# zqqqqz2000/MixGRPO

Measured on AMD Instinct MI355X. Metric: GRPO train-step images/sec, FLUX.1-dev 1024^2, higher is better.
Workload: dtype bf16

## Files before the change

mixgrpo_amd/csrc/attention_bwd.hip:

```cpp
#include "../../include/mixgrpo_hip.h"
#include "attn_fp8_quant.h"
#include "attn_operands.h"
#include "common.h"

#include <cstdlib>
#include <type_traits>

namespace {

constexpr int HD = 128;

__device__ __forceinline__ int rm_off(int row, int chunk) { return row * 256 + ((chunk ^ (row & 15)) << 4); }
__device__ __forceinline__ int t64_off(int d, int slot) { return d * 128 + ((slot ^ ((d >> 1) & 7)) << 4); }
__device__ __forceinline__ int t32_off(int d, int slot) { return d * 64 + ((slot ^ (((d >> 2) ^ (d >> 1)) & 3)) << 4); }

typedef __attribute__((ext_vector_type(4))) unsigned int u32x4;
__device__ __forceinline__ auto buf_rsrc(const void* p, long bytes) {
  const unsigned n = bytes > 0xfffffff0L ? 0xfffffff0u : (unsigned)bytes;
  return __builtin_amdgcn_make_buffer_rsrc(const_cast<void*>(p), 0, (int)n, 0x00020000);
}
template <typename R>
__device__ __forceinline__ uint4 buf_ld16(R rs, unsigned voff, unsigned soff) {
  const u32x4 v = __builtin_amdgcn_raw_buffer_load_b128(rs, (int)voff, (int)soff, 0);
  return make_uint4(v.x, v.y, v.z, v.w);
}
template <typename R>
__device__ __forceinline__ float buf_ld_f32(R rs, unsigned voff, unsigned soff) {
  return __builtin_bit_cast(float, __builtin_amdgcn_raw_buffer_load_b32(rs, (int)voff, (int)soff, 0));
}

__global__ void __launch_bounds__(256) attn_bwd_prep_kernel(const bf16_raw* __restrict__ O, const bf16_raw* __restrict__ dO,
                                                            long ldo, long o_bstride, float* __restrict__ delta,
                                                            bf16_raw* __restrict__ dOt, int H, int S, int Sp, int valid) {
  __shared__ bf16_raw tile[64][130];
  const int lane = threadIdx.x & 63, w = threadIdx.x >> 6;
  const int hh = blockIdx.y, b = blockIdx.z, t0 = blockIdx.x * 64;
  for (int i = 0; i < 16; ++i) {
    const int tl = w * 16 + i, s = t0 + tl;
    uint32_t ud = 0;
    float acc = 0.f;
    if (s < valid) {
      const long off = (long)b * o_bstride + (long)s * ldo + hh * HD + 2 * lane;
      ud = *reinterpret_cast<const uint32_t*>(dO + off);
      const uint32_t uo = *reinterpret_cast<const uint32_t*>(O + off);
      acc = bf2f(ud & 0xffff) * bf2f(uo & 0xffff) + bf2f(ud >> 16) * bf2f(uo >> 16);
    }
    *reinterpret_cast<uint32_t*>(&tile[tl][2 * lane]) = ud;
    acc = wave_sum(acc);
    if (lane == 0 && s < S) delta[((long)b * H + hh) * S + s] = acc;
  }
  __syncthreads();
  for (int id = threadIdx.x; id < 128 * 8; id += 256) {
    const int d = id >> 3, c = id & 7;
    bf16_raw* dst = dOt + (((long)b * H + hh) * HD + d) * Sp + t0 + c * 8;
    if (t0 + c * 8 < Sp) {
      uint4 u;
      u.x = (uint32_t)tile[c * 8 + 0][d] | ((uint32_t)tile[c * 8 + 1][d] << 16);
      u.y = (uint32_t)tile[c * 8 + 2][d] | ((uint32_t)tile[c * 8 + 3][d] << 16);
      u.z = (uint32_t)tile[c * 8 + 4][d] | ((uint32_t)tile[c * 8 + 5][d] << 16);
      u.w = (uint32_t)tile[c * 8 + 6][d] | ((uint32_t)tile[c * 8 + 7][d] << 16);
      *reinterpret_cast<uint4*>(dst) = u;
    }
  }
}

struct BwdArgs {
  const bf16_raw* Q;
  const bf16_raw* K;
  const bf16_raw* V;
  const bf16_raw* Qt;
  const bf16_raw* Kt;
  const bf16_raw* dO;
  const bf16_raw* dOt;
  const float* lse;
  const float* delta;
  bf16_raw* dQ;
  bf16_raw* dK;
  bf16_raw* dV;
  int B, H, S, Sp;
  long ldo, o_bstride;
  float scale, scale_log2e, neg_inv_scale;
  int kv_len;
};

constexpr int DKV_STAGE = 4 * 8192 + 256;
__global__ void __launch_bounds__(512, 2) attn_bwd_dkv_kernel(BwdArgs g) {
  extern __shared__ __attribute__((aligned(16))) char smem[];
  const int tid = threadIdx.x, lane = tid & 63, wid = tid >> 6;
  const int r = lane & 31, h = lane >> 5;
  const int nkb = (g.S + 255) / 256;
  int bid = blockIdx.x;
  xcd_remap(bid, nkb * g.H * g.B);
  const int kt = bid % nkb, bh = bid / nkb;
  const int b = bh / g.H, hh = bh - b * g.H;
  const long bhS = (long)bh * g.S;
  const bf16_raw* Qp = g.Q + bhS * HD;
  const bf16_raw* Qtp = g.Qt + (long)bh * HD * g.Sp;
  const bf16_raw* dOtp = g.dOt + (long)bh * HD * g.Sp;
  const bf16_raw* dOp = g.dO + (long)b * g.o_bstride + hh * HD;

  const int key0 = kt * 256 + wid * 32;
  int krow = key0 + r;
  const bool key_valid = krow < g.S;
  if (krow >= g.S) krow = g.S - 1;
  s16x8 kf[8];
  char* vfrag = smem + 2 * DKV_STAGE + wid * 8192 + lane * 16;
#pragma unroll
  for (int ks = 0; ks < 8; ++ks) {
    kf[ks] = *reinterpret_cast<const s16x8*>(g.K + (bhS + krow) * HD + ks * 16 + h * 8);
    *reinterpret_cast<s16x8*>(vfrag + ks * 1024) =
        *reinterpret_cast<const s16x8*>(g.V + (bhS + krow) * HD + ks * 16 + h * 8);
  }
  f32x16 dv[4], dk[4];
#pragma unroll
  for (int dt = 0; dt < 4; ++dt)
#pragma unroll
    for (int i = 0; i < 16; ++i) dv[dt][i] = dk[dt][i] = 0.f;

  const int s_row = tid >> 4, s_chunk = tid & 15;
  const int s_d = tid >> 2, s_c16 = tid & 3;
  uint4 rq, rdo, rqt, rdot;
  float rl = 0.f;
  const int nqt = (g.S + 31) / 32;
  const auto rs_q = buf_rsrc(Qp, (long)g.S * HD * 2);
  const auto rs_do = buf_rsrc(dOp, ((long)(g.S - 1) * g.ldo + HD) * 2);
  const auto rs_qt = buf_rsrc(Qtp, (long)HD * g.Sp * 2);
  const auto rs_dot = buf_rsrc(dOtp, (long)HD * g.Sp * 2);
  const auto rs_lse = buf_rsrc(g.lse + bhS, (long)g.S * 4);
  const auto rs_dlt = buf_rsrc(g.delta + bhS, (long)g.S * 4);
  const unsigned vo_q = (unsigned)(s_row * HD + s_chunk * 8) * 2, vo_do = (unsigned)(s_row * g.ldo + s_chunk * 8) * 2;
  const unsigned vo_t = (unsigned)(s_d * g.Sp + s_c16 * 8) * 2, vo_l = (unsigned)(tid & 31) * 4;
  float rl2 = 0.f;
  const bool wave0 = __builtin_amdgcn_readfirstlane(wid) == 0;
  const float inv_scale = 1.0f / g.scale;
#define DKV_LOAD(t)                                                                                   \
  do {                                                                                                \
    const unsigned q_base = (unsigned)(t) * 32;                                                       \
    rq = buf_ld16(rs_q, vo_q, q_base * (HD * 2));                                                     \
    rdo = buf_ld16(rs_do, vo_do, q_base * (unsigned)(g.ldo * 2));                                     \
    rqt = buf_ld16(rs_qt, vo_t, q_base * 2);                                                          \
    rdot = buf_ld16(rs_dot, vo_t, q_base * 2);                                                        \
                                                          \
    if (wave0) {           \
      rl = buf_ld_f32(rs_lse, vo_l, q_base * 4);                                                      \
      rl2 = buf_ld_f32(rs_dlt, vo_l, q_base * 4);                                                     \
    }                                                                                                 \
  } while (0)
#define DKV_STORE(buf)                                                                                \
  do {                                                                                                \
    char* base = smem + (buf) * DKV_STAGE;                                                            \
    *reinterpret_cast<uint4*>(base + rm_off(s_row, s_chunk)) = rq;                                    \
    *reinterpret_cast<uint4*>(base + 8192 + rm_off(s_row, s_chunk)) = rdo;                            \
     \
    *reinterpret_cast<uint2*>(base + 16384 + t32_off(s_d, (s_c16 >> 1) * 2) + (s_c16 & 1) * 8) = make_uint2(rqt.x, rqt.y);     \
    *reinterpret_cast<uint2*>(base + 16384 + t32_off(s_d, (s_c16 >> 1) * 2 + 1) + (s_c16 & 1) * 8) = make_uint2(rqt.z, rqt.w); \
    *reinterpret_cast<uint2*>(base + 24576 + t32_off(s_d, (s_c16 >> 1) * 2) + (s_c16 & 1) * 8) = make_uint2(rdot.x, rdot.y);   \
    *reinterpret_cast<uint2*>(base + 24576 + t32_off(s_d, (s_c16 >> 1) * 2 + 1) + (s_c16 & 1) * 8) = make_uint2(rdot.z, rdot.w); \
      \
    if (wave0)                                                                                        \
      reinterpret_cast<float*>(base + 32768)[tid] =                                                   \
          (tid < 32) ? ((nt_ * 32 + tid < g.S) ? -rl * inv_scale : -INFINITY) : -rl2;                 \
  } while (0)

  DKV_LOAD(0);
  { const int nt_ = 0; DKV_STORE(0); }
  __syncthreads();
#pragma unroll
  for (int ks = 0; ks < 8; ++ks) asm volatile("" :: "v"(kf[ks]));
  int cur = 0;
  auto tile = [&](int t, auto mask_tag) __attribute__((always_inline)) {
    constexpr bool MASK = decltype(mask_tag)::value;
    const char* base = smem + cur * DKV_STAGE;
    const float* nls = reinterpret_cast<const float*>(base + 32768);
    const float* ndl = nls + 32;
    f32x16 s, dp;
#pragma unroll
    for (int j = 0; j < 4; ++j) {
      const float4 a = *reinterpret_cast<const float4*>(nls + 8 * j + 4 * h);
      const float4 b2 = *reinterpret_cast<const float4*>(ndl + 8 * j + 4 * h);
      s[4 * j] = a.x; s[4 * j + 1] = a.y; s[4 * j + 2] = a.z; s[4 * j + 3] = a.w;
      dp[4 * j] = b2.x; dp[4 * j + 1] = b2.y; dp[4 * j + 2] = b2.z; dp[4 * j + 3] = b2.w;
    }
    {
      s16x8 qa[2], da[2], vk;
      qa[0] = *reinterpret_cast<const s16x8*>(base + rm_off(r, h));
      da[0] = *reinterpret_cast<const s16x8*>(base + 8192 + rm_off(r, h));
#pragma unroll
      for (int ks = 0; ks < 8; ++ks) {
        vk = *reinterpret_cast<const s16x8*>(vfrag + ks * 1024);
        if (ks + 1 < 8) {
          qa[(ks + 1) & 1] = *reinterpret_cast<const s16x8*>(base + rm_off(r, (ks + 1) * 2 + h));
          da[(ks + 1) & 1] = *reinterpret_cast<const s16x8*>(base + 8192 + rm_off(r, (ks + 1) * 2 + h));
        }
        __builtin_amdgcn_sched_barrier(0);
        s = __builtin_amdgcn_mfma_f32_32x32x16_bf16(qa[ks & 1], kf[ks], s, 0, 0, 0);
        dp = __builtin_amdgcn_mfma_f32_32x32x16_bf16(da[ks & 1], vk, dp, 0, 0, 0);
        __builtin_amdgcn_sched_barrier(0);
      }
    }
    if (t + 1 < nqt) DKV_LOAD(t + 1);
    uint32_t pb[8], dsb[8];
#pragma unroll
    for (int i = 0; i < 16; i += 2) {
      float p0 = __builtin_amdgcn_exp2f(s[i] * g.scale_log2e);
      float p1 = __builtin_amdgcn_exp2f(s[i + 1] * g.scale_log2e);
      if (MASK && !key_valid) p0 = p1 = 0.f;
      const float d0 = p0 * dp[i] * g.scale;
      const float d1 = p1 * dp[i + 1] * g.scale;
      pb[i >> 1] = pack_bf16(p0, p1);
      dsb[i >> 1] = pack_bf16(d0, d1);
    }
    {
      s16x8 pf[2], df[2];
#pragma unroll
      for (int s2 = 0; s2 < 2; ++s2) {
        pf[s2] = __builtin_bit_cast(s16x8, make_uint4(pb[4 * s2], pb[4 * s2 + 1], pb[4 * s2 + 2], pb[4 * s2 + 3]));
        df[s2] = __builtin_bit_cast(s16x8, make_uint4(dsb[4 * s2], dsb[4 * s2 + 1], dsb[4 * s2 + 2], dsb[4 * s2 + 3]));
      }
      auto frag = [&](int i) __attribute__((always_inline)) {
        const int s2 = i >> 3, dt = (i >> 1) & 3, which = i & 1;
        return *reinterpret_cast<const s16x8*>(base + (which ? 16384 : 24576) + t32_off(dt * 32 + r, s2 * 2 + h));
      };
      s16x8 fr[3];
      fr[0] = frag(0); fr[1] = frag(1);
#pragma unroll
      for (int i = 0; i < 16; ++i) {
        if (i + 2 < 16) fr[(i + 2) % 3] = frag(i + 2);
        __builtin_amdgcn_sched_barrier(0);
        const int s2 = i >> 3, dt = (i >> 1) & 3;
        if (i & 1) dk[dt] = __builtin_amdgcn_mfma_f32_32x32x16_bf16(fr[i % 3], df[s2], dk[dt], 0, 0, 0);
        else dv[dt] = __builtin_amdgcn_mfma_f32_32x32x16_bf16(fr[i % 3], pf[s2], dv[dt], 0, 0, 0);
        __builtin_amdgcn_sched_barrier(0);
      }
    }
    if (t + 1 < nqt) { const int nt_ = t + 1; DKV_STORE(cur ^ 1); }
    __syncthreads();
    cur ^= 1;
  };
  if (key0 + 32 > g.S) {
    for (int t = 0; t < nqt; ++t) tile(t, std::true_type{});
  } else {
    for (int t = 0; t < nqt; ++t) tile(t, std::false_type{});
  }
  const int key = key0 + r;
  if (key < g.S) {
    bf16_raw* dkp = g.dK + (bhS + key) * HD;
    bf16_raw* dvp = g.dV + (bhS + key) * HD;
#pragma unroll
    for (int dt = 0; dt < 4; ++dt)
#pragma unroll
      for (int i4 = 0; i4 < 4; ++i4) {
        const int d = dt * 32 + 8 * i4 + 4 * h;
        *reinterpret_cast<uint2*>(dkp + d) = make_uint2(pack_bf16(dk[dt][4 * i4], dk[dt][4 * i4 + 1]),
                                                        pack_bf16(dk[dt][4 * i4 + 2], dk[dt][4 * i4 + 3]));
        *reinterpret_cast<uint2*>(dvp + d) = make_uint2(pack_bf16(dv[dt][4 * i4], dv[dt][4 * i4 + 1]),
                                                        pack_bf16(dv[dt][4 * i4 + 2], dv[dt][4 * i4 + 3]));
      }
  }
}

constexpr int DQ_STAGE = 3 * 16384;
__global__ void __launch_bounds__(512, 2) attn_bwd_dq_kernel(BwdArgs g) {
  extern __shared__ __attribute__((aligned(16))) char smem[];
  const int tid = threadIdx.x, lane = tid & 63, wid = tid >> 6;
  const int r = lane & 31, h = lane >> 5;
  const int nq = (g.S + 255) / 256;
  int bid = blockIdx.x;
  xcd_remap(bid, nq * g.H * g.B);
  const int qt = bid % nq, bh = bid / nq;
  const int b = bh / g.H, hh = bh - b * g.H;
  const long bhS = (long)bh * g.S;
  const bf16_raw* Kp = g.K + bhS * HD;
  const bf16_raw* Vp = g.V + bhS * HD;
  const bf16_raw* Ktp = g.Kt + (long)bh * HD * g.Sp;

  const int q0 = qt * 256 + wid * 32;
  int qrow = q0 + r;
  const bool q_valid = qrow < g.S;
  if (qrow >= g.S) qrow = g.S - 1;
  s16x8 qf[8], dof[8];
  const bf16_raw* dOp = g.dO + (long)b * g.o_bstride + (long)qrow * g.ldo + hh * HD;
#pragma unroll
  for (int ks = 0; ks < 8; ++ks) {
    qf[ks] = *reinterpret_cast<const s16x8*>(g.Q + (bhS + qrow) * HD + ks * 16 + h * 8);
    dof[ks] = *reinterpret_cast<const s16x8*>(dOp + ks * 16 + h * 8);
  }
  const float lse2 = g.lse[bhS + qrow] * 1.4426950408889634f;
  const float dlt = g.delta[bhS + qrow];
  f32x16 dq[4];
#pragma unroll
  for (int dt = 0; dt < 4; ++dt)
#pragma unroll
    for (int i = 0; i < 16; ++i) dq[dt][i] = 0.f;

  const int kc_key0 = tid >> 4, kc_chunk = tid & 15;
  const int vc_d0 = tid >> 3, vc_chunk = tid & 7;
  uint4 sk0, sk1, sv0, sv1, st0, st1;
  const int ntiles = (g.S + 63) / 64;
  const auto rs_k = buf_rsrc(Kp, (long)g.S * HD * 2);
  const auto rs_v = buf_rsrc(Vp, (long)g.S * HD * 2);
  const auto rs_kt = buf_rsrc(Ktp, (long)HD * g.Sp * 2);
  const unsigned vo_k = (unsigned)(kc_key0 * HD + kc_chunk * 8) * 2, vo_kt = (unsigned)(vc_d0 * g.Sp + vc_chunk * 8) * 2;
#define DQ_LOAD(t)                                                                                  \
  do {                                                                                              \
    const unsigned key_base = (unsigned)(t) * 64;                                                   \
    sk0 = buf_ld16(rs_k, vo_k, key_base * (HD * 2));                                                \
    sk1 = buf_ld16(rs_k, vo_k, (key_base + 32) * (HD * 2));                                         \
    sv0 = buf_ld16(rs_v, vo_k, key_base * (HD * 2));                                                \
    sv1 = buf_ld16(rs_v, vo_k, (key_base + 32) * (HD * 2));                                         \
    st0 = buf_ld16(rs_kt, vo_kt, key_base * 2);                                                     \
    st1 = buf_ld16(rs_kt, vo_kt + (unsigned)(64 * g.Sp * 2), key_base * 2);                         \
  } while (0)
#define DQ_STORE(buf)                                                                               \
  do {                                                                                              \
    char* base = smem + (buf) * DQ_STAGE;                                                           \
    *reinterpret_cast<uint4*>(base + rm_off(kc_key0, kc_chunk)) = sk0;                              \
    *reinterpret_cast<uint4*>(base + rm_off(kc_key0 + 32, kc_chunk)) = sk1;                         \
    *reinterpret_cast<uint4*>(base + 16384 + rm_off(kc_key0, kc_chunk)) = sv0;                      \
    *reinterpret_cast<uint4*>(base + 16384 + rm_off(kc_key0 + 32, kc_chunk)) = sv1;                 \
     \
    *reinterpret_cast<uint2*>(base + 32768 + t64_off(vc_d0, (vc_chunk >> 1) * 2) + (vc_chunk & 1) * 8) = make_uint2(st0.x, st0.y); \
    *reinterpret_cast<uint2*>(base + 32768 + t64_off(vc_d0, (vc_chunk >> 1) * 2 + 1) + (vc_chunk & 1) * 8) = make_uint2(st0.z, st0.w); \
    *reinterpret_cast<uint2*>(base + 32768 + t64_off(vc_d0 + 64, (vc_chunk >> 1) * 2) + (vc_chunk & 1) * 8) = make_uint2(st1.x, st1.y); \
    *reinterpret_cast<uint2*>(base + 32768 + t64_off(vc_d0 + 64, (vc_chunk >> 1) * 2 + 1) + (vc_chunk & 1) * 8) = make_uint2(st1.z, st1.w); \
  } while (0)

  DQ_LOAD(0);
  DQ_STORE(0);
  __syncthreads();
#pragma unroll
  for (int ks = 0; ks < 8; ++ks) asm volatile("" :: "v"(qf[ks]), "v"(dof[ks]));
  asm volatile("" :: "v"(lse2), "v"(dlt));
  int cur = 0;
  auto tile = [&](int t, auto mask_tag) __attribute__((always_inline)) {
    constexpr bool MASK = decltype(mask_tag)::value;
    if (t + 1 < ntiles) DQ_LOAD(t + 1);
    const char* base = smem + cur * DQ_STAGE;
    const int key_base = t * 64;
#pragma unroll
    for (int kb = 0; kb < 2; ++kb) {
      f32x16 s, dp;
#pragma unroll
      for (int i = 0; i < 16; ++i) s[i] = dp[i] = 0.f;
      {
        s16x8 ka[3], va[3];
#pragma unroll
        for (int ks = 0; ks < 2; ++ks) {
          ka[ks] = *reinterpret_cast<const s16x8*>(base + rm_off(kb * 32 + r, ks * 2 + h));
          va[ks] = *reinterpret_cast<const s16x8*>(base + 16384 + rm_off(kb * 32 + r, ks * 2 + h));
        }
#pragma unroll
        for (int ks = 0; ks < 8; ++ks) {
          if (ks + 2 < 8) {
            ka[(ks + 2) % 3] = *reinterpret_cast<const s16x8*>(base + rm_off(kb * 32 + r, (ks + 2) * 2 + h));
            va[(ks + 2) % 3] = *reinterpret_cast<const s16x8*>(base + 16384 + rm_off(kb * 32 + r, (ks + 2) * 2 + h));
          }
          __builtin_amdgcn_sched_barrier(0);
          s = __builtin_amdgcn_mfma_f32_32x32x16_bf16(ka[ks % 3], qf[ks], s, 0, 0, 0);
          dp = __builtin_amdgcn_mfma_f32_32x32x16_bf16(va[ks % 3], dof[ks], dp, 0, 0, 0);
          __builtin_amdgcn_sched_barrier(0);
        }
      }
      uint32_t dsb[8];
#pragma unroll
      for (int i = 0; i < 16; i += 2) {
        const int k0 = key_base + kb * 32 + (i & 3) + 8 * (i >> 2) + 4 * h;
        float p0 = __builtin_amdgcn_exp2f(s[i] * g.scale_log2e - lse2);
        float p1 = __builtin_amdgcn_exp2f(s[i + 1] * g.scale_log2e - lse2);
        if (MASK) {
          if (k0 >= g.S) p0 = 0.f;
          if (k0 + 1 >= g.S) p1 = 0.f;
        }
        dsb[i >> 1] = pack_bf16(p0 * (dp[i] - dlt) * g.scale, p1 * (dp[i + 1] - dlt) * g.scale);
      }
      {
        s16x8 df[2];
#pragma unroll
        for (int s2 = 0; s2 < 2; ++s2)
          df[s2] = __builtin_bit_cast(s16x8, make_uint4(dsb[4 * s2], dsb[4 * s2 + 1], dsb[4 * s2 + 2], dsb[4 * s2 + 3]));
        auto frag = [&](int i) __attribute__((always_inline)) {
          return *reinterpret_cast<const s16x8*>(base + 32768 + t64_off((i & 3) * 32 + r, (kb * 2 + (i >> 2)) * 2 + h));
        };
        s16x8 fr[4];
        fr[0] = frag(0); fr[1] = frag(1); fr[2] = frag(2);
#pragma unroll
        for (int i = 0; i < 8; ++i) {
          if (i + 3 < 8) fr[(i + 3) & 3] = frag(i + 3);
          __builtin_amdgcn_sched_barrier(0);
          dq[i & 3] = __builtin_amdgcn_mfma_f32_32x32x16_bf16(fr[i & 3], df[i >> 2], dq[i & 3], 0, 0, 0);
          __builtin_amdgcn_sched_barrier(0);
        }
      }
    }
    if (t + 1 < ntiles) DQ_STORE(cur ^ 1);
    __syncthreads();
    cur ^= 1;
  };
  const int nfull = g.S / 64;
  for (int t = 0; t < nfull; ++t) tile(t, std::false_type{});
  if (nfull < ntiles) tile(nfull, std::true_type{});
  if (q_valid) {
    bf16_raw* dqp = g.dQ + (bhS + q0 + r) * HD;
#pragma unroll
    for (int dt = 0; dt < 4; ++dt)
#pragma unroll
      for (int i4 = 0; i4 < 4; ++i4) {
        const int d = dt * 32 + 8 * i4 + 4 * h;
        *reinterpret_cast<uint2*>(dqp + d) = make_uint2(pack_bf16(dq[dt][4 * i4], dq[dt][4 * i4 + 1]),
                                                        pack_bf16(dq[dt][4 * i4 + 2], dq[dt][4 * i4 + 3]));
      }
  }
}

#include "attn_bwd_dq64_body.inc"
#include "attn_bwd_dq64kv_body.inc"
#include "attn_bwd_dkv64_body.inc"
#include "attn_bwd_dkv64kv_body.inc"

#define LO(x) "s"((unsigned)(x))
#define HI(x) "s"((unsigned)((x) >> 32))
#define UNIFORM(x) "s"(__builtin_amdgcn_readfirstlane(x))

#define ATTN_BWD_DQ64_OPERANDS                                                                                                  \
  [tid] "v"(threadIdx.x), [q_lo] LO(qp), [q_hi] HI(qp), [k_lo] LO(kp), [k_hi] HI(kp), [v_lo] LO(vp), [v_hi] HI(vp),              \
      [kt_lo] LO(ktp), [kt_hi] HI(ktp), [do_lo] LO(dop), [do_hi] HI(dop), [lse_lo] LO(lsep), [lse_hi] HI(lsep), [dl_lo] LO(dlp), \
      [dl_hi] HI(dlp), [dq_lo] LO(dqp), [dq_hi] HI(dqp), [sp2] "s"(g.Sp * 2), [ldo2] "s"((int)(g.ldo * 2)),                      \
      [cs] "s"(g.scale_log2e), [scale] "s"(g.scale), [nloop] "s"(ops.nloop), [seq] "s"(ops.seq)
#define ATTN_BWD_DQ64_KV_OPERANDS ATTN_BWD_DQ64_OPERANDS, [kt0] UNIFORM(ops.kt0), [kt1] UNIFORM(ops.kt1), [qlast] UNIFORM(ops.qlast)

template <bool KV>
__global__ void __launch_bounds__(256, 1) attn_bwd_dq64_kernel(BwdArgs g) {
  const int nq = g.S >> 8;
  int bid = blockIdx.x;
  xcd_remap(bid, nq * g.H * g.B);
  const int qt = bid % nq, bh = bid / nq;
  const int b = bh / g.H, hh = bh - b * g.H;
  const long bhS = (long)bh * g.S;
  const unsigned long long qp = (unsigned long long)(g.Q + (bhS + qt * 256) * HD);
  const unsigned long long kp = (unsigned long long)(g.K + bhS * HD);
  const unsigned long long vp = (unsigned long long)(g.V + bhS * HD);
  const unsigned long long ktp = (unsigned long long)(g.Kt + (long)bh * HD * g.Sp);
  const unsigned long long dop = (unsigned long long)(g.dO + (long)b * g.o_bstride + (long)(qt * 256) * g.ldo + hh * HD);
  const unsigned long long lsep = (unsigned long long)(g.lse + bhS + qt * 256);
  const unsigned long long dlp = (unsigned long long)(g.delta + bhS + qt * 256);
  const unsigned long long dqp = (unsigned long long)(g.dQ + (bhS + qt * 256) * HD);
  const attn_ops::Dq64 ops = attn_ops::dq64(KV, g.S, g.kv_len, qt);
  if constexpr (KV) asm volatile(ATTN_BWD_DQ64KV_BODY : : ATTN_BWD_DQ64_KV_OPERANDS : ATTN_BWD_DQ64KV_CLOBBERS);
  else asm volatile(ATTN_BWD_DQ64_BODY : : ATTN_BWD_DQ64_OPERANDS : ATTN_BWD_DQ64_CLOBBERS);
}

#define ATTN_BWD_DKV64_OPERANDS                                                                                                \
  [tid] "v"(threadIdx.x), [q_lo] LO(qp), [q_hi] HI(qp), [do_lo] LO(dop), [do_hi] HI(dop), [qt_lo] LO(qtp), [qt_hi] HI(qtp),     \
      [dot_lo] LO(dotp), [dot_hi] HI(dotp), [k_lo] LO(kp), [k_hi] HI(kp), [v_lo] LO(vp), [v_hi] HI(vp), [lse_lo] LO(lsep),      \
      [lse_hi] HI(lsep), [dl_lo] LO(dlp), [dl_hi] HI(dlp), [dk_lo] LO(dkp), [dk_hi] HI(dkp), [dv_lo] LO(dvp), [dv_hi] HI(dvp),  \
      [sp2] "s"(g.Sp * 2), [ldo2] "s"((int)(g.ldo * 2)), [cs] "s"(g.scale_log2e), [scale] "s"(g.scale),                         \
      [nis] "s"(g.neg_inv_scale), [nloop] "s"(ops.nloop), [qmax] "s"(ops.qmax), [ldo32] "s"((int)(g.ldo * 64)), [cmax] "s"(ops.cmax)
#define ATTN_BWD_DKV64_KV_OPERANDS ATTN_BWD_DKV64_OPERANDS, [qk] UNIFORM(ops.qk), [klast] UNIFORM(ops.klast)

template <bool KV>
__global__ void __launch_bounds__(256, 1) attn_bwd_dkv64_kernel(BwdArgs g) {
  const int nkb = g.S >> 8;
  int bid = blockIdx.x;
  xcd_remap(bid, nkb * g.H * g.B);
  const int kt = bid % nkb, bh = bid / nkb;
  const int b = bh / g.H, hh = bh - b * g.H;
  const long bhS = (long)bh * g.S;
  const unsigned long long qp = (unsigned long long)(g.Q + bhS * HD);
  const unsigned long long dop = (unsigned long long)(g.dO + (long)b * g.o_bstride + hh * HD);
  const unsigned long long qtp = (unsigned long long)(g.Qt + (long)bh * HD * g.Sp);
  const unsigned long long dotp = (unsigned long long)(g.dOt + (long)bh * HD * g.Sp);
  const unsigned long long kp = (unsigned long long)(g.K + (bhS + kt * 256) * HD);
  const unsigned long long vp = (unsigned long long)(g.V + (bhS + kt * 256) * HD);
  const unsigned long long lsep = (unsigned long long)(g.lse + bhS);
  const unsigned long long dlp = (unsigned long long)(g.delta + bhS);
  const unsigned long long dkp = (unsigned long long)(g.dK + (bhS + kt * 256) * HD);
  const unsigned long long dvp = (unsigned long long)(g.dV + (bhS + kt * 256) * HD);
  const attn_ops::Dkv64 ops = attn_ops::dkv64(KV, g.S, g.kv_len, kt);
  if constexpr (KV) asm volatile(ATTN_BWD_DKV64KV_BODY : : ATTN_BWD_DKV64_KV_OPERANDS : ATTN_BWD_DKV64KV_CLOBBERS);
  else asm volatile(ATTN_BWD_DKV64_BODY : : ATTN_BWD_DKV64_OPERANDS : ATTN_BWD_DKV64_CLOBBERS);
}

#undef LO
#undef HI
#undef UNIFORM
}

static bool attn_bwd_wide(int B, int H, int S, int Sp, long ldo, long o_bstride) {
  const char* w64e = getenv("MGX_ATTN_W64");
  const int w64 = w64e ? atoi(w64e) : 1;
  return w64 && S % 256 == 0 && Sp == S && ldo * 2 * 256 < (1L << 31) && ldo * 2 < (1L << 24) && Sp * 2 < (1L << 24);
}

static bool attn_bwd_kv_wide(int B, int H, int Sa, int kv_len, long ldo, long o_bstride) {
  return B > 0 && H > 0 && Sa > 0 && kv_len > Sa - 256 && kv_len <= Sa && o_bstride >= (long)Sa * ldo &&
         attn_bwd_wide(B, H, Sa, Sa, ldo, o_bstride);
}

static int attn_bwd_begin(BwdArgs& g, const uint16_t* Q, const uint16_t* K, const uint16_t* V, const uint16_t* Qt,
                          const uint16_t* Kt, const uint16_t* O, const uint16_t* dO, const float* lse, float* delta, uint16_t* dOt,
                          uint16_t* dQ, uint16_t* dK, uint16_t* dV, int B, int H, int S, int Sp, int kv_len, long ldo,
                          long o_bstride, float scale, bool taken, hipStream_t st) {
  MGX_REQUIRE(Q && K && V && Qt && Kt && O && dO && lse && delta && dOt && dQ && dK && dV, "null operand");
  MGX_REQUIRE(ldo % 8 == 0 && o_bstride % 8 == 0, "dO rows must be 16-byte aligned");
  if (!taken) return 1;
  MGX_REQUIRE(B > 0 && H > 0 && S > 0 && Sp >= S && Sp % 64 == 0, "bad sizes");
  g.Q = Q; g.K = K; g.V = V; g.Qt = Qt; g.Kt = Kt; g.dO = dO; g.dOt = dOt; g.lse = lse; g.delta = delta;
  g.dQ = dQ; g.dK = dK; g.dV = dV; g.B = B; g.H = H; g.S = S; g.Sp = Sp; g.ldo = ldo; g.o_bstride = o_bstride;
  g.scale = scale; g.scale_log2e = scale * 1.4426950408889634f; g.neg_inv_scale = -1.0f / scale;
  g.kv_len = kv_len;
  attn_bwd_prep_kernel<<<dim3(Sp / 64, H, B), 256, 0, st>>>(O, dO, ldo, o_bstride, delta, dOt, H, S, Sp, kv_len);
  return MGX_OK;
}

void mgx_attn_bwd_prep_launch(const uint16_t* O, const uint16_t* dO, long ldo, long o_bstride, float* delta, uint16_t* dOt,
                              int B, int H, int S, int Sp, hipStream_t st) {
  attn_bwd_prep_kernel<<<dim3(Sp / 64, H, B), 256, 0, st>>>(O, dO, ldo, o_bstride, delta, dOt, H, S, Sp, S);
}

extern "C" int mgx_attn_bwd(const uint16_t* Q, const uint16_t* K, const uint16_t* V, const uint16_t* Qt, const uint16_t* Kt,
                            const uint16_t* O, const uint16_t* dO, const float* lse, float* delta, uint16_t* dOt,
                            uint16_t* dQ, uint16_t* dK, uint16_t* dV, int B, int H, int S, int Sp, long ldo, long o_bstride,
                            float scale, void* stream) {
  hipStream_t st = (hipStream_t)stream;
  BwdArgs g;
  if (const int rc = attn_bwd_begin(g, Q, K, V, Qt, Kt, O, dO, lse, delta, dOt, dQ, dK, dV, B, H, S, Sp, S, ldo, o_bstride, scale,
                                    true, st))
    return rc;
  const int nb = cdiv(S, 256) * H * B;
  if (attn_bwd_wide(B, H, S, Sp, ldo, o_bstride)) {
    launch_lds<attn_bwd_dkv64_kernel<false>, 149504>(nb, 256, st, g);
    launch_lds<attn_bwd_dq64_kernel<false>, 98304>(nb, 256, st, g);
  } else {
    launch_lds<attn_bwd_dkv_kernel, 2 * DKV_STAGE + 65536>(nb, 512, st, g);
    launch_lds<attn_bwd_dq_kernel, 2 * DQ_STAGE>(nb, 512, st, g);
  }
  MGX_CHECK_LAUNCH();
  return MGX_OK;
}

extern "C" int mgx_attn_bwd_path(int B, int H, int S, int Sp, long ldo, long o_bstride) {
  MGX_REQUIRE(B > 0 && H > 0 && S > 0 && Sp >= S && Sp % 64 == 0, "bad sizes");
  return attn_bwd_wide(B, H, S, Sp, ldo, o_bstride) ? 1 : 0;
}

extern "C" int mgx_attn_bwd_kv(const uint16_t* Q, const uint16_t* K, const uint16_t* V, const uint16_t* Qt, const uint16_t* Kt,
                               const uint16_t* O, const uint16_t* dO, const float* lse, float* delta, uint16_t* dOt,
                               uint16_t* dQ, uint16_t* dK, uint16_t* dV, int B, int H, int Sa, int kv_len, long ldo,
                               long o_bstride, float scale, void* stream) {
  hipStream_t st = (hipStream_t)stream;
  BwdArgs g;
  if (const int rc = attn_bwd_begin(g, Q, K, V, Qt, Kt, O, dO, lse, delta, dOt, dQ, dK, dV, B, H, Sa, Sa, kv_len, ldo, o_bstride,
                                    scale, attn_bwd_kv_wide(B, H, Sa, kv_len, ldo, o_bstride), st))
    return rc;
  const int nb = (Sa / 256) * H * B;
  launch_lds<attn_bwd_dkv64_kernel<true>, 149504>(nb, 256, st, g);
  launch_lds<attn_bwd_dq64_kernel<true>, 98304>(nb, 256, st, g);
  MGX_CHECK_LAUNCH();
  return MGX_OK;
}

extern "C" int mgx_attn_bwd_kv_path(int B, int H, int Sa, int kv_len, long ldo, long o_bstride) {
  return attn_bwd_kv_wide(B, H, Sa, kv_len, ldo, o_bstride) ? 1 : 0;
}
```

Baseline: 0.4536.

## Run attention backward 64-wide kernels as persistent grid-stride workgroups

Turns the dK/dV and dQ 64-wide backward kernels into persistent kernels: a fixed grid (default 256 workgroups, overridable by MGX_ATTN_BWD_GRID) loops over virtual block indices, with an s_barrier handover between iterations. The aim is to cut workgroup launch and tail-scheduling overhead and keep one resident workgroup per CU. In exchange, load balance now depends on the grid size, and back-to-back blocks on a workgroup run serially with extra barriers. An A/B timing script is added under scratch.

```diff
diff --git a/mixgrpo_amd/csrc/attention_bwd.hip b/mixgrpo_amd/csrc/attention_bwd.hip
--- a/mixgrpo_amd/csrc/attention_bwd.hip
+++ b/mixgrpo_amd/csrc/attention_bwd.hip
@@ -412,6 +412,8 @@
   }
 }
 
+#define ATTN_BWD_HANDOVER() asm volatile("s_barrier" ::: "memory")
+
 #include "attn_bwd_dq64_body.inc"
 #include "attn_bwd_dq64kv_body.inc"
 #include "attn_bwd_dkv64_body.inc"
@@ -429,10 +431,10 @@
 #define ATTN_BWD_DQ64_KV_OPERANDS ATTN_BWD_DQ64_OPERANDS, [kt0] UNIFORM(ops.kt0), [kt1] UNIFORM(ops.kt1), [qlast] UNIFORM(ops.qlast)
 
 template <bool KV>
-__global__ void __launch_bounds__(256, 1) attn_bwd_dq64_kernel(BwdArgs g) {
+__device__ __forceinline__ void attn_bwd_dq64_block(const BwdArgs& g, int vb, int nb) {
   const int nq = g.S >> 8;
-  int bid = blockIdx.x;
-  xcd_remap(bid, nq * g.H * g.B);
+  int bid = vb;
+  xcd_remap(bid, nb);
   const int qt = bid % nq, bh = bid / nq;
   const int b = bh / g.H, hh = bh - b * g.H;
   const long bhS = (long)bh * g.S;
@@ -447,6 +449,13 @@
   const attn_ops::Dq64 ops = attn_ops::dq64(KV, g.S, g.kv_len, qt);
   if constexpr (KV) asm volatile(ATTN_BWD_DQ64KV_BODY : : ATTN_BWD_DQ64_KV_OPERANDS : ATTN_BWD_DQ64KV_CLOBBERS);
   else asm volatile(ATTN_BWD_DQ64_BODY : : ATTN_BWD_DQ64_OPERANDS : ATTN_BWD_DQ64_CLOBBERS);
+  ATTN_BWD_HANDOVER();
+}
+
+template <bool KV>
+__global__ void __launch_bounds__(256, 1) attn_bwd_dq64_kernel(BwdArgs g) {
+  const int nb = (g.S >> 8) * g.H * g.B;
+  for (int vb = blockIdx.x; vb < nb; vb += gridDim.x) attn_bwd_dq64_block<KV>(g, vb, nb);
 }
 
 #define ATTN_BWD_DKV64_OPERANDS                                                                                                \
@@ -458,10 +467,10 @@
 #define ATTN_BWD_DKV64_KV_OPERANDS ATTN_BWD_DKV64_OPERANDS, [qk] UNIFORM(ops.qk), [klast] UNIFORM(ops.klast)
 
 template <bool KV>
-__global__ void __launch_bounds__(256, 1) attn_bwd_dkv64_kernel(BwdArgs g) {
+__device__ __forceinline__ void attn_bwd_dkv64_block(const BwdArgs& g, int vb, int nb) {
   const int nkb = g.S >> 8;
-  int bid = blockIdx.x;
-  xcd_remap(bid, nkb * g.H * g.B);
+  int bid = vb;
+  xcd_remap(bid, nb);
   const int kt = bid % nkb, bh = bid / nkb;
   const int b = bh / g.H, hh = bh - b * g.H;
   const long bhS = (long)bh * g.S;
@@ -478,8 +487,16 @@
   const attn_ops::Dkv64 ops = attn_ops::dkv64(KV, g.S, g.kv_len, kt);
   if constexpr (KV) asm volatile(ATTN_BWD_DKV64KV_BODY : : ATTN_BWD_DKV64_KV_OPERANDS : ATTN_BWD_DKV64KV_CLOBBERS);
   else asm volatile(ATTN_BWD_DKV64_BODY : : ATTN_BWD_DKV64_OPERANDS : ATTN_BWD_DKV64_CLOBBERS);
-}
-
+  ATTN_BWD_HANDOVER();
+}
+
+template <bool KV>
+__global__ void __launch_bounds__(256, 1) attn_bwd_dkv64_kernel(BwdArgs g) {
+  const int nb = (g.S >> 8) * g.H * g.B;
+  for (int vb = blockIdx.x; vb < nb; vb += gridDim.x) attn_bwd_dkv64_block<KV>(g, vb, nb);
+}
+
+#undef ATTN_BWD_HANDOVER
 #undef LO
 #undef HI
 #undef UNIFORM
@@ -489,6 +506,19 @@
   const char* w64e = getenv("MGX_ATTN_W64");
   const int w64 = w64e ? atoi(w64e) : 1;
   return w64 && S % 256 == 0 && Sp == S && ldo * 2 * 256 < (1L << 31) && ldo * 2 < (1L << 24) && Sp * 2 < (1L << 24);
+}
+
+static int attn_bwd_grid(int blocks) {
+  const char* e = getenv("MGX_ATTN_BWD_GRID");
+  const int want = e ? atoi(e) : 256;
+  return want < 1 ? 1 : want > blocks ? blocks : want;
+}
+
+template <bool KV>
+static void attn_bwd_launch64(const BwdArgs& g, int nb, hipStream_t st) {
+  const int grid = attn_bwd_grid(nb);
+  launch_lds<attn_bwd_dkv64_kernel<KV>, 149504>(grid, 256, st, g);
+  launch_lds<attn_bwd_dq64_kernel<KV>, 98304>(grid, 256, st, g);
 }
 
 static bool attn_bwd_kv_wide(int B, int H, int Sa, int kv_len, long ldo, long o_bstride) {
@@ -528,8 +558,7 @@
     return rc;
   const int nb = cdiv(S, 256) * H * B;
   if (attn_bwd_wide(B, H, S, Sp, ldo, o_bstride)) {
-    launch_lds<attn_bwd_dkv64_kernel<false>, 149504>(nb, 256, st, g);
-    launch_lds<attn_bwd_dq64_kernel<false>, 98304>(nb, 256, st, g);
+    attn_bwd_launch64<false>(g, nb, st);
   } else {
     launch_lds<attn_bwd_dkv_kernel, 2 * DKV_STAGE + 65536>(nb, 512, st, g);
     launch_lds<attn_bwd_dq_kernel, 2 * DQ_STAGE>(nb, 512, st, g);
@@ -553,8 +582,7 @@
                                     scale, attn_bwd_kv_wide(B, H, Sa, kv_len, ldo, o_bstride), st))
     return rc;
   const int nb = (Sa / 256) * H * B;
-  launch_lds<attn_bwd_dkv64_kernel<true>, 149504>(nb, 256, st, g);
-  launch_lds<attn_bwd_dq64_kernel<true>, 98304>(nb, 256, st, g);
+  attn_bwd_launch64<true>(g, nb, st);
   MGX_CHECK_LAUNCH();
   return MGX_OK;
 }
diff --git a/scratch/ab_attn_bwd_walk.py b/scratch/ab_attn_bwd_walk.py
--- /dev/null
+++ b/scratch/ab_attn_bwd_walk.py
@@ -0,0 +1,70 @@
+import ctypes as C, math, os, statistics, sys, torch
+sys.path.insert(0, ".")
+from mixgrpo_amd import _lib
+new = _lib.lib()
+old = C.CDLL(os.path.join("scratch", "libmixgrpo_parent.so"))
+res, args = _lib.SIGNATURES["mgx_attn_bwd"]
+old.mgx_attn_bwd.restype, old.mgx_attn_bwd.argtypes = res, args
+REPS = int(sys.argv[1]) if len(sys.argv) > 1 else 7
+N = int(sys.argv[2]) if len(sys.argv) > 2 else 10
+B, H, S = 4, 24, 4608
+st = torch.cuda.current_stream().cuda_stream
+for mult in (1, 5):
+    torch.manual_seed(0)
+    ldo = H * 128 * mult
+    q, k, v = (torch.randn(B, H, S, 128, device="cuda").bfloat16() for _ in range(3))
+    q2 = (q.float() * (1.4426950408889634 / math.sqrt(128))).bfloat16()
+    qt, kt = q2.transpose(-1, -2).contiguous(), k.transpose(-1, -2).contiguous()
+    sc = (q2.float() @ k.float().transpose(-1, -2)) * math.log(2.0)
+    lse = torch.logsumexp(sc, -1)
+    o = (torch.softmax(sc, -1) @ v.float()).bfloat16()
+    del sc
+    Ofull = torch.zeros(B, S, ldo, device="cuda", dtype=torch.bfloat16)
+    dOfull = torch.randn(B, S, ldo, device="cuda").bfloat16()
+    Ofull[:, :, :H * 128] = o.permute(0, 2, 1, 3).reshape(B, S, H * 128)
+    outs = {}
+    for name in ("old", "new"):
+        outs[name] = dict(delta=torch.empty(B, H, S, device="cuda"), dOt=torch.empty(B, H, 128, S, device="cuda", dtype=torch.bfloat16),
+                          **{n: torch.empty(B, H, S, 128, device="cuda", dtype=torch.bfloat16) for n in ("dQ", "dK", "dV")})
+
+    def call(lib, o_):
+        rc = lib.mgx_attn_bwd(q2.data_ptr(), k.data_ptr(), v.data_ptr(), qt.data_ptr(), kt.data_ptr(), Ofull.data_ptr(), dOfull.data_ptr(),
+                              lse.data_ptr(), o_["delta"].data_ptr(), o_["dOt"].data_ptr(), o_["dQ"].data_ptr(), o_["dK"].data_ptr(),
+                              o_["dV"].data_ptr(), B, H, S, S, ldo, S * ldo, math.log(2.0), st)
+        assert rc == 0
+
+    def t(lib, o_, **env):
+        os.environ.pop("MGX_ATTN_BWD_GRID", None)
+        os.environ.update({key: str(val) for key, val in env.items()})
+        call(lib, o_); torch.cuda.synchronize()
+        e0, e1 = torch.cuda.Event(enable_timing=True), torch.cuda.Event(enable_timing=True)
+        e0.record()
+        for _ in range(N): call(lib, o_)
+        e1.record(); torch.cuda.synchronize()
+        for key in env:
+            os.environ.pop(key, None)
+        return e0.elapsed_time(e1) / N
+
+    call(old, outs["old"]); call(new, outs["new"]); torch.cuda.synchronize()
+    same = all(torch.equal(outs["old"][n].view(torch.int16 if outs["old"][n].element_size() == 2 else torch.int32),
+                           outs["new"][n].view(torch.int16 if outs["new"][n].element_size() == 2 else torch.int32)) for n in outs["old"])
+    print(f"ldo = {mult} d: outputs of the two libraries bit-identical (dQ, dK, dV, delta, dOt): {same}", flush=True)
+    assert same
+    assert all(bool(torch.isfinite(x.float()).all()) for x in outs["new"].values())
+    blocks = B * H * S // 256
+    for _ in range(2):
+        t(old, outs["old"]); t(new, outs["new"])
+    rows = {"parent": [], "walk (256 workgroups)": [], f"this build, one block per workgroup ({blocks})": []}
+    for rep in range(REPS):
+        a, b, c = t(old, outs["old"]), t(new, outs["new"]), t(new, outs["new"], MGX_ATTN_BWD_GRID=blocks)
+        for key, x in zip(rows, (a, b, c)):
+            rows[key].append(x)
+        print(f"  rep {rep}: parent {a:.4f} ms   walk {b:.4f} ms   one-block {c:.4f} ms", flush=True)
+    for key, xs in rows.items():
+        print(f"  {key}: median {statistics.median(xs):.4f} ms, span {max(xs) - min(xs):.4f} ms ({min(xs):.4f} .. {max(xs):.4f})")
+    m = {key: statistics.median(xs) for key, xs in rows.items()}
+    span = max(max(xs) - min(xs) for xs in list(rows.values())[:2])
+    gain = m["parent"] - m["walk (256 workgroups)"]
+    print(f"  parent - walk = {gain:.4f} ms ({100 * gain / m['parent']:.2f} %), 3 x the larger span = {3 * span:.4f} ms", flush=True)
+    del q, k, v, q2, qt, kt, lse, o, Ofull, dOfull, outs
+    torch.cuda.empty_cache()
```

Result: no change. 0.4540 (median of 4 runs) (+0.1%).
